# ai4ce/V2X-Sim

Measured on AMD Instinct MI355X. Metric: BEV frames/sec, V2VNet 5-agent detection (256x256 BEV), higher is better.
Workload: dtype bf16

## Files before the change

v2x-sim_amd/csrc/conv_stream.hip:

```cpp
#include "conv_stream.h"
#include <cstdlib>
#include <type_traits>



#ifndef V2X_STREAM_PSWZ_BUILD
#define V2X_STREAM_PSWZ_BUILD 1
#endif
constexpr int PSH = V2X_STREAM_PSWZ_BUILD;
#ifndef V2X_STREAM_LSS_BUILD
#define V2X_STREAM_LSS_BUILD 1
#endif

template <int BCO>
constexpr int chain_lds_bytes() { return BCO * BCO * 2 + 2 * BCO * 4; }

template <int BCO, int NT>
__device__ __forceinline__ void stage_chain(const StreamArgs &a, char *cl) {
    constexpr int NKS = BCO / 32;
    for (int p = threadIdx.x; p < BCO * BCO / 8; p += NT) {
        const int row = p / (BCO / 8), c8 = p - row * (BCO / 8);
        const int i2 = row >> 4, fj = row & 15, ks = c8 >> 2, fq = c8 & 3;
        *reinterpret_cast<uint4 *>(cl + (((i2 * NKS + ks) * 4 + fq) * 16 + fj) * 16) =
            *reinterpret_cast<const uint4 *>(a.w2 + (size_t)row * BCO + c8 * 8);
// ... 305 lines not shown
        const bool first = kc < nc0;
        const bool hf = first && a.up0;
        int d = hf ? pd_half[0] : pd_full[0];
#pragma unroll
        for (int u = 1; u < 6; ++u) d = (t == u) ? (hf ? pd_half[u] : pd_full[u]) : d;
        glds16s(patch_src(a.in0, a.C0, a.in1, a.C1, nc0, kc, zero_page, d), s_patch + buf * PATCH_BYTES + (wave + 4 * t) * 1024);
    };
    auto issue_dummy = [&]() { glds16s(zero_page, s_dummy); };

#pragma unroll
    for (int t = 0; t < 6; ++t) issue_patch_piece(kc_lo, t, 0);
    issue_weights(0);
    issue_weights(1);
    issue_weights(2);

    f32x4_t acc[TCO][4];
#pragma unroll
    for (int i = 0; i < TCO; ++i)
#pragma unroll
        for (int f = 0; f < 4; ++f) acc[i][f] = (f32x4_t){0.f, 0.f, 0.f, 0.f};

    int s = 0;
    for (int kc = kc_lo; kc < kc_hi; ++kc) {
        const char *pb = s_patch + ((kc - kc_lo) & 1) * PATCH_BYTES;
        const bool half = (kc < nc0) && a.up0;
        const int sh = half ? 1 : 0, row_bytes = (half ? PW0 : PW) * 64;
#pragma unroll 1
        for (int ky = 0; ky < 3; ++ky) {
            int rowoff[4];
#pragma unroll
            for (int f = 0; f < 4; ++f) rowoff[f] = (((frow[f] + ky - sh) >> sh) + sh) * row_bytes;
#pragma unroll
            for (int kx = 0; kx < 3; ++kx, ++s) {
                const int tap = ky * 3 + kx;
                if (s + 3 >= S) wait_vmcnt<0>();
                else if (s < 2) { if (NW == 2) wait_vmcnt<4>(); else wait_vmcnt<2>(); }
                else { if (NW == 2) wait_vmcnt<6>(); else wait_vmcnt<4>(); }
                __builtin_amdgcn_s_barrier();
                if (s + 3 < S) {
                    issue_weights(s + 3);
                    if (tap < 6 && kc + 1 < kc_hi) issue_patch_piece(kc + 1, tap, (kc + 1 - kc_lo) & 1);
                    else issue_dummy();
                }
                const char *ws = s_ring + (s & (RING - 1)) * SLICE_BYTES;
                bf16x8_t fa[TCO], fb[4];
#pragma unroll
                for (int f = 0; f < 4; ++f)
                    fb[f] = *reinterpret_cast<const bf16x8_t *>(pb + rowoff[f] + (half ? ct_half[f][kx] : ct_full[f][kx]));
#pragma unroll
                for (int i = 0; i < TCO; ++i)
                    fa[i] = *reinterpret_cast<const bf16x8_t *>(ws + (fq * BCO + i * 16 + fj) * 16);
#pragma unroll
                for (int i = 0; i < TCO; ++i)
#pragma unroll
                    for (int f = 0; f < 4; ++f)
                        acc[i][f] = __builtin_amdgcn_mfma_f32_16x16x32_bf16(fa[i], fb[f], acc[i][f], 0, 0, 0);

                __builtin_amdgcn_sched_group_barrier(0x100, TCO + 4, 0);
                __builtin_amdgcn_sched_group_barrier(0x008, TCO * 4, 0);
            }
        }
    }

    if constexpr (SPLITK) {
        const size_t npix = (size_t)a.N * a.H * a.W;
#pragma unroll
        for (int i = 0; i < TCO; ++i)
#pragma unroll
            for (int f = 0; f < 4; ++f) {
                const size_t pix = (size_t)(n * a.H + y0 + frow[f]) * a.W + x0 + ((TW == 32) ? (f & 1) * 16 + fj : fj);
                *reinterpret_cast<f32x4_t *>(a.ws + ((size_t)blockIdx.y * npix + pix) * a.w_rows + co_tile * BCO + i * 16 + fq * 4) = acc[i][f];
            }
    } else {
        stream_epilogue<BCO, TW, EPI, 4, false, true, true>(a, acc, co_tile, n, y0, x0, frow, fj, fq, nullptr, nullptr, 0, a.x4 != 0);
    }
}

template <bool GRU>
__global__ __launch_bounds__(256) void splitk_reduce_kernel(const float *__restrict__ ws, int ksplit, long long npix, int w_rows, int Cout,
                                                            const float *__restrict__ scale, const float *__restrict__ shift, int relu,
                                                            uint16_t *__restrict__ out, int out_cstride, int out_coff) {
    const int quads = Cout / 4;
    const long long total = npix * quads;
    for (long long t = (long long)blockIdx.x * 256 + threadIdx.x; t < total; t += (long long)gridDim.x * 256) {
        const long long pix = t / quads;
        const int c = (int)(t - pix * quads) * 4;
        if constexpr (GRU) {
            const int row = (c >> 5) * 96 + ((c >> 4) & 1) * 48 + (c & 15);
            f32x4_t g[3];
#pragma unroll
            for (int q = 0; q < 3; ++q) g[q] = (f32x4_t){0.f, 0.f, 0.f, 0.f};
            for (int sp = 0; sp < ksplit; ++sp)
#pragma unroll
                for (int q = 0; q < 3; ++q) g[q] += *reinterpret_cast<const f32x4_t *>(ws + ((size_t)sp * npix + pix) * w_rows + row + 16 * q);
            float h[4];
#pragma unroll
            for (int r = 0; r < 4; ++r) {
                const float4 b = reinterpret_cast<const float4 *>(scale)[c + r];
                h[r] = v2x_gru_h0(g[0][r], g[1][r], g[2][r], b);
            }
            uint2 o;
            o.x = pack_bf16x2(h[0], h[1]);
            o.y = pack_bf16x2(h[2], h[3]);
            *reinterpret_cast<uint2 *>(out + pix * out_cstride + out_coff + c) = o;
        } else {
            f32x4_t v = (f32x4_t){0.f, 0.f, 0.f, 0.f};
            for (int sp = 0; sp < ksplit; ++sp) v += *reinterpret_cast<const f32x4_t *>(ws + ((size_t)sp * npix + pix) * w_rows + c);
            const float4 sc = *reinterpret_cast<const float4 *>(scale + c), sf = *reinterpret_cast<const float4 *>(shift + c);
            uint2 o;
            o.x = pack_bf16x2(v[0] * sc.x + sf.x, v[1] * sc.y + sf.y);
            o.y = pack_bf16x2(v[2] * sc.z + sf.z, v[3] * sc.w + sf.w);
            if (relu) {
                o.x = v2x_relu_bf16x2(o.x);
                o.y = v2x_relu_bf16x2(o.y);
            }
            *reinterpret_cast<uint2 *>(out + pix * out_cstride + out_coff + c) = o;
        }
    }
}


template <int BCO, int EPI>
__global__ __launch_bounds__(512) __attribute__((amdgpu_waves_per_eu(2, 2))) void conv3x3_stream8_kernel(const StreamArgs a) {
    constexpr bool PERSIST = (EPI != SEPI_CHAIN);
    constexpr int TH = 16, TW = 32;
    constexpr int PW = TW + 2, PH = TH + 2, PW0 = TW / 2 + 2;
    constexpr int TCO = BCO / 16;
    constexpr int W_PIECES = BCO / 16;
    constexpr int SLICE_BYTES = BCO * 64;
    constexpr int N_ST = (EPI == SEPI_GRU) ? (TCO / 3) * 4 : TCO * 4;
    static_assert(PH * PW * 4 <= (PATCH8_PIECES - 1) * 64, "patch must leave the last piece as padding");
    static_assert(W_PIECES <= 8, "at most one weight DMA per wave per step");
    static_assert(4 + N_ST <= 63, "vmcnt is a 6-bit counter");

    extern __shared__ __attribute__((aligned(16))) char smem[];
    char *s_ring = smem;
    char *s_patch = smem + RING * SLICE_BYTES;
    char *s_dummy = s_patch + (PATCH8_PIECES - 1) * 1024;

    const int tid = threadIdx.x;
    const int lane = tid & 63;
    const int wave = __builtin_amdgcn_readfirstlane(tid >> 6);
    const int grp = wave >> 2, wv = wave & 3;
    const int fj = lane & 15, fq = lane >> 4;

    const int nwg = gridDim.x;
    const int bid = xcd_major_bid(blockIdx.x, nwg);
    const int n_tiles = a.n_px_tiles * a.n_co_tiles;
    const int co_tile = bid % a.n_co_tiles;
    const int txy = a.tiles_x * a.tiles_y;

    const int nc0 = a.C0 >> 5, nchunks = (a.C0 + a.C1) >> 5;
    const int S = nchunks * 9;
    const uint16_t *wbase = a.w + (size_t)co_tile * nchunks * 9 * (BCO * 32);
    const void *zero_page = a.w + (size_t)a.n_co_tiles * nchunks * 9 * (BCO * 32);
    char *s_chain = smem + RING * SLICE_BYTES + 2 * PATCH8_BYTES;
    if constexpr (EPI == SEPI_CHAIN) stage_chain<BCO, 512>(a, s_chain);

    auto tile_coords = [&](int t, int &n, int &y0, int &x0) { stream_tile_coords<TH, TW>(a.tiles_x, a.n_co_tiles, txy, t, n, y0, x0); };
    auto desc = [&](int n, int y0, int x0, int t, bool hf) -> int {
        return patch_desc<TH, TW, PSH>(a.H, a.W, n, y0, x0, (wave + 8 * t) * 64 + lane, hf);
    };

    int frow[4], ct[4][3];
#pragma unroll
    for (int f = 0; f < 4; ++f) frow[f] = 8 * grp + 2 * wv + (f >> 1);

    const bool has_w = wave < W_PIECES;
    const uint16_t *wsrc = wbase + lane * 8 + wave * 512;
    auto issue_dummy = [&]() { glds16s(zero_page, s_dummy); };
    auto issue_slice = [&](int slice, int slot, bool real) {
        if (has_w && real) glds16s(wsrc + (size_t)slice * (BCO * 32), s_ring + slot * SLICE_BYTES + wave * 1024);
        else issue_dummy();
    };
    auto issue_piece = [&](int d, int kc, int t, int buf) {
        glds16s(patch_src(a.in0, a.C0, a.in1, a.C1, nc0, kc, zero_page, d), s_patch + buf * PATCH8_BYTES + (wave + 8 * t) * 1024);
    };
    const bool chunk0_half = (nc0 > 0) && a.up0;

    int tile = bid;
    int n, y0, x0;
    tile_coords(tile, n, y0, x0);
    int pd[5];
    bool pd_half = chunk0_half;
#pragma unroll
    for (int t = 0; t < 5; ++t) pd[t] = desc(n, y0, x0, t, pd_half);

#pragma unroll
    for (int t = 0; t < 5; ++t) issue_piece(pd[t], 0, t, 0);
    issue_slice(0, 0, true); issue_dummy();
    issue_slice(1, 1, true); issue_dummy();
    issue_slice(2, 2, true); issue_dummy();
    wait_vmcnt<4>();
    __builtin_amdgcn_s_barrier();
    if (grp == 1) __builtin_amdgcn_s_barrier();

    int g = 0;
    int gc = 0;
    int relaxed = 0;
    for (;;) {
        const int next = tile + nwg;
        const bool has_next = PERSIST && next < n_tiles;
        int nn = 0, ny0 = 0, nx0 = 0;
        if (has_next) tile_coords(next, nn, ny0, nx0);

        f32x4_t acc[TCO][4];
#pragma unroll
        for (int i = 0; i < TCO; ++i)
#pragma unroll
            for (int f = 0; f < 4; ++f) acc[i][f] = (f32x4_t){0.f, 0.f, 0.f, 0.f};

        int s = 0;
        for (int kc = 0; kc < nchunks; ++kc, ++gc) {
            const char *pb = s_patch + (gc & 1) * PATCH8_BYTES;
            const bool half = (kc < nc0) && a.up0;
            const int sh = half ? 1 : 0, row_bytes = (half ? PW0 : PW) * 64;
            const bool last_chunk = kc + 1 == nchunks;
            const int kcn = last_chunk ? 0 : kc + 1;
            const bool fill = !last_chunk || has_next;
            const bool hfn = (kcn < nc0) && a.up0;
            if ((last_chunk && has_next) || (fill && hfn != pd_half)) {
                const int dn = last_chunk ? nn : n, dy = last_chunk ? ny0 : y0, dx = last_chunk ? nx0 : x0;
#pragma unroll
                for (int t = 0; t < 5; ++t) {
                    pd[t] = desc(dn, dy, dx, t, hfn);
                    __builtin_amdgcn_sched_barrier(0);
                }
                pd_half = hfn;
            }
            if (kc == 0 || kc == nc0) patch_col_table<4, TW, PSH>(ct, fj, fq, half);
#pragma unroll 1
            for (int ky = 0; ky < 3; ++ky) {
                int rowoff[4];
#pragma unroll
                for (int f = 0; f < 4; ++f) rowoff[f] = (((frow[f] + ky - sh) >> sh) + sh) * row_bytes;
#pragma unroll
                for (int kx = 0; kx < 3; ++kx, ++s, ++g) {
                    const int tap = ky * 3 + kx;
                    {
                        const int s3 = s + 3;
                        issue_slice(s3 < S ? s3 : s3 - S, (g + 3) & (RING - 1), s3 < S || has_next);
                    }
                    if (tap < 5 && fill) {
                        int d = pd[0];
#pragma unroll
                        for (int u = 1; u < 5; ++u) d = (tap == u) ? pd[u] : d;
                        issue_piece(d, kcn, tap, (gc + 1) & 1);
                    } else {
                        issue_dummy();
                    }
                    const char *ws = s_ring + (g & (RING - 1)) * SLICE_BYTES;
                    bf16x8_t fa[TCO], fb[4];
#pragma unroll
                    for (int f = 0; f < 4; ++f)
                        fb[f] = *reinterpret_cast<const bf16x8_t *>(pb + rowoff[f] + ct[f][kx]);
#pragma unroll
                    for (int i = 0; i < TCO; ++i)
                        fa[i] = *reinterpret_cast<const bf16x8_t *>(ws + (fq * BCO + i * 16 + fj) * 16);
                    if (relaxed > 0) {
                        wait_vmcnt<4 + N_ST>();
                        --relaxed;
                    } else {
                        wait_vmcnt<4>();
                    }
                    asm volatile("s_waitcnt lgkmcnt(0)" ::: "memory");
                    __builtin_amdgcn_sched_barrier(0);
                    __builtin_amdgcn_s_barrier();
                    __builtin_amdgcn_sched_barrier(0);
#pragma unroll
                    for (int i = 0; i < TCO; ++i)
#pragma unroll
                        for (int f = 0; f < 4; ++f)
                            acc[i][f] = __builtin_amdgcn_mfma_f32_16x16x32_bf16(fa[i], fb[f], acc[i][f], 0, 0, 0);
                    __builtin_amdgcn_sched_barrier(0);
                    __builtin_amdgcn_s_barrier();
                    __builtin_amdgcn_sched_barrier(0);
                }
            }
        }
        stream_epilogue<BCO, TW, EPI, 4, EPI == SEPI_CHAIN, true, EPI == SEPI_CHAIN>(a, acc, co_tile, n, y0, x0, frow, fj, fq, s_chain, nullptr, 0, a.x4 != 0);
        if (!has_next) break;
        tile = next;
        n = nn;
        y0 = ny0;
        x0 = nx0;
        relaxed = 2;
    }
    if (grp == 0) __builtin_amdgcn_s_barrier();
}

int v2x_conv_stream_pc_launch(const StreamArgs &a, hipStream_t s);

int v2x_num_cus() {
    static int n[V2X_MAX_DEVICES] = {0};
    int dev = 0, v = 0;
    if (hipGetDevice(&dev) != hipSuccess || dev < 0 || dev >= V2X_MAX_DEVICES) return 256;
    if (n[dev] == 0)
        n[dev] = (hipDeviceGetAttribute(&v, hipDeviceAttributeMultiprocessorCount, dev) == hipSuccess && v > 0) ? v : 256;
    return n[dev];
}

#define V2X_STREAM8G_ISSUE_DMAS \
                if (grp == 1) { \
                    const int ahead = st + 2; \
                    const int wslot = slot == 0 ? 2 : slot - 1; \
                    if (ahead < S3) nw = issue_weights(ahead, wslot, wv, 4); \
                    else if (has_next && ahead - S3 < S3) nw = issue_weights(ahead - S3, wslot, wv, 4); \
                } else if (fill && kx < 2) { \
                    const int npieces = hfn ? (PH0 * PW0 * 4 + 63) / 64 : PATCH8_PIECES; \
_Pragma("unroll") \
                    for (int t = 0; t < 5; ++t) { \
                        const int tt = kx * 5 + t; \
                        if (wv + 4 * tt >= npieces) break; \
                        int d = pd[0]; \
_Pragma("unroll") \
                        for (int u = 1; u < 10; ++u) d = (tt == u) ? pd[u] : d; \
                        issue_piece(d, kcn, tt, (gc + 1) & 1); \
                    } \
                }
template <int BCO, int EPI, bool WT = false>
__global__ __launch_bounds__(512) __attribute__((amdgpu_waves_per_eu(2, 2))) void conv3x3_stream8g_kernel(const StreamArgs a) {
    constexpr int TH = 16, TW = 32;
    constexpr int PW = TW + 2, PH = TH + 2, PW0 = TW / 2 + 2, PH0 = TH / 2 + 2;
    constexpr int TCO = BCO / 16, HCO = TCO / 2;
    constexpr int W_PIECES = BCO / 16;
    constexpr int SLICE_BYTES = BCO * 64;
    constexpr int STEP_BYTES = 3 * SLICE_BYTES;
    constexpr int NWD = (3 * W_PIECES + 3) / 4;
    static_assert(EPI != SEPI_CHAIN, "the chained epilogue stays on conv3x3_stream8_kernel (its operands need the LDS; from L2: +5.3 %)");
    static_assert(TCO % 2 == 0 && PH * PW * 4 <= (PATCH8_PIECES - 1) * 64, "half taps; patch fits its buffer");
    constexpr int AT = WT ? HCO : TCO;
    constexpr int NF = WT ? 8 : 4;
    constexpr int NB = WT ? 12 : 8;
    constexpr int BT = (HCO % 2 == 0) ? 2 : HCO;
    constexpr int N_ST = (EPI == SEPI_GRU) ? (TCO / 3) * 2 : TCO * 2;

    extern __shared__ __attribute__((aligned(16))) char smem[];
    char *s_ring = smem;
    char *s_patch = smem + 3 * STEP_BYTES;

    const int tid = threadIdx.x;
    const int lane = tid & 63;
    const int wave = __builtin_amdgcn_readfirstlane(tid >> 6);
    const int grp = wave >> 2, wv = wave & 3;
    const int fj = lane & 15, fq = lane >> 4;

    const int nwg = gridDim.x;
    int bid = xcd_major_bid(blockIdx.x, nwg);
    if (a.xcd_walk != 0 && a.n_co_tiles == 8 && (nwg & 7) == 0 && (nwg >> 3) == 32) {
        const int x = bid >> 5, i = bid & 31;
        bid = (((x >> 1) * 8 + (i >> 2)) << 3) + (x & 1) * 4 + (i & 3);
    }
    const int n_tiles = a.n_px_tiles * a.n_co_tiles;
    const int co_tile = bid % a.n_co_tiles;
    const int txy = a.tiles_x * a.tiles_y;
    const int nc0 = a.C0 >> 5, nchunks = (a.C0 + a.C1) >> 5;
    const int S3 = nchunks * 3;
    const uint16_t *wbase = a.w + (size_t)co_tile * nchunks * 9 * (BCO * 32);
    const void *zero_page = a.w + (size_t)a.n_co_tiles * nchunks * 9 * (BCO * 32);

    auto tile_coords = [&](int t, int &n, int &y0, int &x0) { stream_tile_coords<TH, TW>(a.tiles_x, a.n_co_tiles, txy, t, n, y0, x0); };
    auto desc = [&](int n, int y0, int x0, int t, bool hf) -> int {
        return patch_desc<TH, TW, PSH>(a.H, a.W, n, y0, x0, (wv + 4 * t) * 64 + fresh_lane(), hf);
    };
    auto issue_piece = [&](int d, int kc, int t, int buf) {
        glds16s_aux<V2X_STREAM8G_PATCH_AUX>(patch_src(a.in0, a.C0, a.in1, a.C1, nc0, kc, zero_page, d), s_patch + buf * PATCH8_BYTES + (wv + 4 * t) * 1024);
    };
    auto issue_weights = [&](int st, int slot, int wq, int NQ) -> int {
        const int kc = st / 3, kx = st - kc * 3;
        const int lane_w = fresh_lane();
        int cnt = 0;
#pragma unroll
        for (int u = 0; u < NWD; ++u) {
            const int p = wq + NQ * u;
            if (p >= 3 * W_PIECES) break;
            ++cnt;
            const int ky = p / W_PIECES, pis = p - ky * W_PIECES;
            glds16s_aux<V2X_STREAM8G_WEIGHT_AUX>(wbase + (size_t)(kc * 9 + ky * 3 + kx) * (BCO * 32) + pis * 512 + lane_w * 8,
                    s_ring + slot * STEP_BYTES + ky * SLICE_BYTES + pis * 1024);
        }
        return cnt;
    };
    auto wait_keep = [&](int keep, bool plus_stores) {
        if (plus_stores) {
            if (keep == NWD) asm volatile("s_waitcnt vmcnt(%0)" ::"n"(NWD + N_ST) : "memory");
            else if (keep == NWD - 1) asm volatile("s_waitcnt vmcnt(%0)" ::"n"(NWD - 1 + N_ST) : "memory");
            else asm volatile("s_waitcnt vmcnt(%0)" ::"n"(N_ST) : "memory");
        } else {
            if (keep == NWD) asm volatile("s_waitcnt vmcnt(%0)" ::"n"(NWD) : "memory");
            else if (keep == NWD - 1) asm volatile("s_waitcnt vmcnt(%0)" ::"n"(NWD - 1) : "memory");
            else asm volatile("s_waitcnt vmcnt(0)" ::: "memory");
        }
    };

    const int coh = WT ? (wv & 1) : 0;
    const int R0 = WT ? 8 * grp + 4 * (wv >> 1) : 8 * grp + 2 * wv;
    int frow[NF];
#pragma unroll
    for (int f = 0; f < NF; ++f) frow[f] = R0 + (f >> 1);
    const bool chunk0_half = (nc0 > 0) && a.up0;

    int tile = bid;
    int n, y0, x0;
    tile_coords(tile, n, y0, x0);
    int pd[10];
    bool pd_half = chunk0_half;
    if (grp == 0) {
#pragma unroll
        for (int t = 0; t < 10; ++t) pd[t] = desc(n, y0, x0, t, pd_half);
#pragma unroll
        for (int t = 0; t < 10; ++t) issue_piece(pd[t], 0, t, 0);
    }
    {
        constexpr int NP8 = (3 * W_PIECES + 7) / 8;
        for (int stp = 0; stp < (S3 > 1 ? 2 : 1); ++stp) {
            const int lane_w = fresh_lane();
#pragma unroll
            for (int u = 0; u < NP8; ++u) {
                const int p = wave + 8 * u;
                if (p >= 3 * W_PIECES) break;
                const int ky = p / W_PIECES, pis = p - ky * W_PIECES;
                glds16s_aux<V2X_STREAM8G_WEIGHT_AUX>(wbase + (size_t)((stp / 3) * 9 + ky * 3 + (stp % 3)) * (BCO * 32) + pis * 512 + lane_w * 8,
                        s_ring + stp * STEP_BYTES + ky * SLICE_BYTES + pis * 1024);
            }
        }
    }
    float *s_ss = reinterpret_cast<float *>(smem + 3 * STEP_BYTES + 2 * PATCH8_BYTES);
    if constexpr (V2X_STREAM_LSS_BUILD != 0 && EPI != SEPI_GRU) {
        if constexpr (EPI == SEPI_GRU) {
            constexpr int NH = BCO / 3;
            for (int i = tid; i < NH * 4; i += 512) {
                const int hc = co_tile * NH + (i >> 2);
                s_ss[i] = hc < a.Cout ? a.scale[(size_t)hc * 4 + (i & 3)] : 0.f;
            }
        } else {
            for (int i = tid; i < BCO; i += 512) {
                const int co = co_tile * BCO + i;
                s_ss[i] = co < a.Cout ? a.scale[co] : 0.f;
                s_ss[BCO + i] = co < a.Cout ? a.shift[co] : 0.f;
            }
        }
    }
    asm volatile("s_waitcnt vmcnt(0) lgkmcnt(0)" ::: "memory");
    __builtin_amdgcn_s_barrier();
    if (grp == 1) __builtin_amdgcn_s_barrier();

    int g = 0;
    bool relaxed = false;
    int slot = 0;
    int gc = 0;
    for (;;) {
        const int next = tile + nwg;
        const bool has_next = next < n_tiles;
        int nn = 0, ny0 = 0, nx0 = 0;
        if (has_next) tile_coords(next, nn, ny0, nx0);

        f32x4_t acc[AT][NF];
#pragma unroll
        for (int i = 0; i < AT; ++i)
#pragma unroll
            for (int f = 0; f < NF; ++f) acc[i][f] = (f32x4_t)(0.f);

        for (int kc = 0; kc < nchunks; ++kc, ++gc) {
            const char *pb = s_patch + (gc & 1) * PATCH8_BYTES;
            const bool half = (kc < nc0) && a.up0;
            const bool last_chunk = kc + 1 == nchunks;
            const int kcn = last_chunk ? 0 : kc + 1;
            const bool fill = !last_chunk || has_next;
            const bool hfn = (kcn < nc0) && a.up0;
            if (grp == 0 && ((last_chunk && has_next) || (fill && hfn != pd_half))) {
                const int dn = last_chunk ? nn : n, dy = last_chunk ? ny0 : y0, dx = last_chunk ? nx0 : x0;
#pragma unroll
                for (int t = 0; t < 10; ++t) {
                    pd[t] = desc(dn, dy, dx, t, hfn);
                    __builtin_amdgcn_sched_barrier(0);
                }
                pd_half = hfn;
            }
            const int sh = half ? 1 : 0;
            const int row_bytes = (half ? PW0 : PW) * 64;
            const int row0 = (R0 >> sh) * row_bytes;
#pragma unroll 1
            for (int kx = 0; kx < 3; ++kx, ++g, slot = (slot == 2 ? 0 : slot + 1)) {
                const int st = kc * 3 + kx;
                const int ln = fresh_lane();
                const int fjl = ln & 15, fql = ln >> 4;
                int nw = 0;
                V2X_STREAM8G_ISSUE_DMAS
                __builtin_amdgcn_sched_barrier(0);
                bf16x8_t B[NB];
#pragma unroll
                for (int ch = 0; ch < 2; ++ch) {
                    const int col = ch * 16 + fjl + kx;
                    const int pc = ((col - sh) >> sh) + sh;
                    const int coff = ((pc << 2) + (fql ^ ((pc >> PSH) & 3))) * 16;
#pragma unroll
                    for (int q = 0; q < NB / 2; ++q) {
                        B[q * 2 + ch] = *reinterpret_cast<const bf16x8_t *>(pb + row0 + (((q - sh) >> sh) + sh) * row_bytes + coff);
                    }
                }
                const char *ws = s_ring + slot * STEP_BYTES + (fql * BCO + fjl) * 16 + coh * (HCO * 256);
                bf16x8_t A[2][WT ? BT : HCO];
#pragma unroll
                for (int i = 0; i < (WT ? BT : HCO); ++i) A[0][i] = *reinterpret_cast<const bf16x8_t *>(ws + i * 256);
                __builtin_amdgcn_s_waitcnt(0xc07f);
                if (grp == 1) {
                    wait_keep(nw, relaxed);
                    relaxed = false;
                } else if (kx == 2) {
                    asm volatile("s_waitcnt vmcnt(0)" ::: "memory");
                }
                __builtin_amdgcn_sched_barrier(0);
                __builtin_amdgcn_s_barrier();
                __builtin_amdgcn_sched_barrier(0);
                if constexpr (WT) {
                    constexpr int NBLK = 3 * HCO / BT;
#pragma unroll
                    for (int b = 0; b < NBLK; ++b) {
                        const int ky = (b * BT) / HCO, i0 = (b * BT) % HCO;
                        auto mma_tiles = [&](int j0, int j1) __attribute__((always_inline)) {
#pragma unroll
                            for (int j = j0; j < j1; ++j)
#pragma unroll
                                for (int f = 0; f < 8; ++f)
                                    acc[i0 + j][f] = __builtin_amdgcn_mfma_f32_16x16x32_bf16(A[b & 1][j], B[((f >> 1) + ky) * 2 + (f & 1)], acc[i0 + j][f], 0, 0, 0);
                        };
                        __builtin_amdgcn_sched_barrier(0);
                        mma_tiles(0, 1);
                        __builtin_amdgcn_sched_barrier(0);
                        if (b + 1 < NBLK) {
                            const int ky1 = ((b + 1) * BT) / HCO, j1 = ((b + 1) * BT) % HCO;
#pragma unroll
                            for (int j = 0; j < BT; ++j) A[(b + 1) & 1][j] = *reinterpret_cast<const bf16x8_t *>(ws + ky1 * SLICE_BYTES + (j1 + j) * 256);
                        }
                        __builtin_amdgcn_sched_barrier(0);
                        mma_tiles(1, BT);
                        __builtin_amdgcn_sched_barrier(0);
                    }
                } else {
                constexpr int H1 = 1;
#pragma unroll
                for (int h = 0; h < 6; ++h) {
                    const int ky = h >> 1, hh = h & 1;
                    auto mma_part = [&](int i0, int i1) __attribute__((always_inline)) {
#pragma unroll
                        for (int i = i0; i < i1; ++i)
#pragma unroll
                            for (int f = 0; f < 4; ++f)
                                acc[hh * HCO + i][f] = __builtin_amdgcn_mfma_f32_16x16x32_bf16(A[h & 1][i], B[((f >> 1) + ky) * 2 + (f & 1)], acc[hh * HCO + i][f], 0, 0, 0);
                    };
                    __builtin_amdgcn_sched_barrier(0);
                    mma_part(0, H1);
                    __builtin_amdgcn_sched_barrier(0);
                    if (h + 1 < 6) {
                        const int ky1 = (h + 1) >> 1, hh1 = (h + 1) & 1;
#pragma unroll
                        for (int i = 0; i < HCO; ++i) A[(h + 1) & 1][i] = *reinterpret_cast<const bf16x8_t *>(ws + ky1 * SLICE_BYTES + (hh1 * HCO + i) * 256);
                    }
                    __builtin_amdgcn_sched_barrier(0);
                    mma_part(H1, HCO);
                    __builtin_amdgcn_sched_barrier(0);
                }
                }
                __builtin_amdgcn_sched_barrier(0);
                __builtin_amdgcn_s_barrier();
                __builtin_amdgcn_sched_barrier(0);
            }
        }
        constexpr bool LSS = V2X_STREAM_LSS_BUILD != 0 && EPI != SEPI_GRU;
        if constexpr (WT)
            stream_epilogue<BCO / 2, TW, EPI, 8, false, true, true>(a, acc, co_tile * 2 + coh, n, y0, x0, frow, fj, fq, nullptr,
                                                                    LSS ? (lds_cf_t *)s_ss + coh * (EPI == SEPI_GRU ? 4 * (BCO / 6) : BCO / 2) : (lds_cf_t *)nullptr, BCO, a.x4 != 0);
        else stream_epilogue<BCO, TW, EPI, 4, false, true, true>(a, acc, co_tile, n, y0, x0, frow, fj, fq, nullptr, LSS ? (lds_cf_t *)s_ss : (lds_cf_t *)nullptr, BCO, a.x4 != 0);
        if (!has_next) break;
        tile = next;
        n = nn;
        y0 = ny0;
        x0 = nx0;
        relaxed = true;
    }
    if (grp == 0) __builtin_amdgcn_s_barrier();
}

template <int BCO, int EPI, bool WT = false>
static int launch_stream8g(const StreamArgs &a, hipStream_t s) {
    constexpr int smem = 3 * 3 * BCO * 64 + 2 * PATCH8_BYTES + 1024;
    static_assert(smem <= 160 * 1024, "LDS budget");
    const int n_tiles = a.n_px_tiles * a.n_co_tiles;
    int grid = n_tiles;
    int g = v2x_num_cus() / a.n_co_tiles * a.n_co_tiles;
    if (g > 0 && g < n_tiles) grid = g;
    return v2x_launch<conv3x3_stream8g_kernel<BCO, EPI, WT>>("conv3x3_stream8g_kernel", dim3(grid), dim3(512), smem, s, a);
}

template <int BCO, int EPI>
static int launch_stream8(const StreamArgs &a, hipStream_t s) {
    constexpr int smem = RING * BCO * 64 + 2 * PATCH8_BYTES + (EPI == SEPI_CHAIN ? chain_lds_bytes<BCO>() : 0);
    const int n_tiles = a.n_px_tiles * a.n_co_tiles;
    int grid = n_tiles;
    if (v2x_tune(V2X_TUNE_STREAM_PERSIST) != 0) {
        int g = v2x_num_cus() / a.n_co_tiles * a.n_co_tiles;
        if (EPI != SEPI_CHAIN && g > 0 && g < n_tiles && ((a.C0 + a.C1) >> 5) >= 2) grid = g;
    }
    return v2x_launch<conv3x3_stream8_kernel<BCO, EPI>>("conv3x3_stream8_kernel", dim3(grid), dim3(512), smem, s, a);
}

constexpr int WPATCH_PIECES = 39;
constexpr int WPATCH_BYTES = WPATCH_PIECES * 1024;

template <int BCO, int EPI>
__global__ __launch_bounds__(256) __attribute__((amdgpu_waves_per_eu(2, 2))) void conv3x3_wide_kernel(const StreamArgs a) {
    constexpr int TH = 16, TW = 32, NF = 8;
    constexpr int PW = TW + 2, PH = TH + 2, PW0 = TW / 2 + 2, PH0 = TH / 2 + 2;
    constexpr int TCO = BCO / 16;
    constexpr int SLICE_BYTES = BCO * 64;
    constexpr int PPW = (WPATCH_PIECES + 3) / 4;
    static_assert(BCO == 64, "wide form: one 64-row channel tile (1 weight DMA per wave and step)");
    static_assert(PH * PW * 4 <= WPATCH_PIECES * 64, "patch must fit its buffer");

    extern __shared__ __attribute__((aligned(16))) char smem[];
    char *s_ring = smem;
    char *s_patch = smem + RING * SLICE_BYTES;

    const int tid = threadIdx.x;
    const int lane = tid & 63;
    const int wave = __builtin_amdgcn_readfirstlane(tid >> 6);
    const int fj = lane & 15, fq = lane >> 4;

    const int bid = xcd_major_bid(blockIdx.x, gridDim.x);
    int co_tile, n, y0, x0;
    stream_tile_coords<TH, TW>(a.tiles_x, a.tiles_y, a.n_co_tiles, bid, co_tile, n, y0, x0);

    const int nc0 = a.C0 >> 5, nchunks = (a.C0 + a.C1) >> 5;
    const int S = nchunks * 9;
    const uint16_t *wbase = a.w + (size_t)co_tile * nchunks * 9 * (BCO * 32);
    const void *zero_page = a.w + (size_t)a.n_co_tiles * nchunks * 9 * (BCO * 32);
    char *s_chain = smem + RING * SLICE_BYTES + WPATCH_BYTES;
    if constexpr (EPI == SEPI_CHAIN) stage_chain<BCO, 256>(a, s_chain);

    int pd[PPW];
    auto build_pd = [&](bool hf) {
        int lane_o = lane;
        asm volatile("" : "+v"(lane_o));
#pragma unroll
        for (int t = 0; t < PPW; ++t) {
            pd[t] = patch_desc<TH, TW, PSH>(a.H, a.W, n, y0, x0, (wave + 4 * t) * 64 + lane_o, hf);
            __builtin_amdgcn_sched_barrier(0);
        }
    };
    int frow[NF], ct[2][3];
#pragma unroll
    for (int f = 0; f < NF; ++f) frow[f] = 4 * wave + (f >> 1);

    const uint16_t *wsrc = wbase + lane * 8 + wave * 512;
    auto issue_weights = [&](int s) {
        glds16s(wsrc + (size_t)s * (BCO * 32), s_ring + (s & (RING - 1)) * SLICE_BYTES + wave * 1024);
    };
    auto issue_patch = [&](int kc, bool hf) {
        const bool first = kc < nc0;
        const uint16_t *src = first ? a.in0 : a.in1;
        const unsigned cs = first ? (unsigned)a.C0 : (unsigned)a.C1;
        const int npieces = hf ? (PH0 * PW0 * 4 + 63) / 64 : WPATCH_PIECES;
#pragma unroll
        for (int t = 0; t < PPW; ++t) {
            if (wave + 4 * t >= npieces) break;
            int d = pd[t];
            asm volatile("" : "+v"(d));
            glds16s(patch_src(src, cs, first ? kc : kc - nc0, zero_page, d), s_patch + (wave + 4 * t) * 1024);
        }
    };

    f32x4_t acc[TCO][NF];
#pragma unroll
    for (int i = 0; i < TCO; ++i)
#pragma unroll
        for (int f = 0; f < NF; ++f) acc[i][f] = (f32x4_t){0.f, 0.f, 0.f, 0.f};

    issue_weights(0);
    issue_weights(1);
    issue_weights(2);

    int s = 0;
    bool cur_half = false;
    for (int kc = 0; kc < nchunks; ++kc) {
        const bool half = (kc < nc0) && a.up0;
        const int sh = half ? 1 : 0, row_bytes = (half ? PW0 : PW) * 64;
        if (kc == 0 || half != cur_half) {
            build_pd(half);
            patch_col_table<2, TW, PSH>(ct, fj, fq, half);
            cur_half = half;
        }
        if (kc > 0) __builtin_amdgcn_s_barrier();
        issue_patch(kc, half);
        wait_vmcnt<0>();
        __builtin_amdgcn_s_barrier();
#pragma unroll 1
        for (int ky = 0; ky < 3; ++ky) {
            int rowoff[NF / 2];
#pragma unroll
            for (int r = 0; r < NF / 2; ++r) rowoff[r] = (((4 * wave + r + ky - sh) >> sh) + sh) * row_bytes;
#pragma unroll
            for (int kx = 0; kx < 3; ++kx, ++s) {
                const int tap = ky * 3 + kx;
                if (tap > 0) {
                    if (s + 2 >= S) wait_vmcnt<0>();
                    else wait_vmcnt<2>();
                    __builtin_amdgcn_s_barrier();
                }
                if (s + 3 < S) issue_weights(s + 3);
                const char *ws = s_ring + (s & (RING - 1)) * SLICE_BYTES;
                bf16x8_t fa[TCO], fb[NF];
#pragma unroll
                for (int f = 0; f < NF; ++f) fb[f] = *reinterpret_cast<const bf16x8_t *>(s_patch + rowoff[f >> 1] + ct[f & 1][kx]);
#pragma unroll
                for (int i = 0; i < TCO; ++i)
                    fa[i] = *reinterpret_cast<const bf16x8_t *>(ws + (fq * BCO + i * 16 + fj) * 16);
#pragma unroll
                for (int i = 0; i < TCO; ++i)
#pragma unroll
                    for (int f = 0; f < NF; ++f)
                        acc[i][f] = __builtin_amdgcn_mfma_f32_16x16x32_bf16(fa[i], fb[f], acc[i][f], 0, 0, 0);
                __builtin_amdgcn_sched_group_barrier(0x100, TCO + NF, 0);
                __builtin_amdgcn_sched_group_barrier(0x008, TCO * NF, 0);
            }
        }
    }
    stream_epilogue<BCO, TW, EPI, NF, EPI == SEPI_CHAIN, true, true>(a, acc, co_tile, n, y0, x0, frow, fj, fq, s_chain, nullptr, 0, a.x4 != 0);
}

template <int BCO>
__global__ __launch_bounds__(256) __attribute__((amdgpu_waves_per_eu(2, 2))) void conv3x3_wide3_kernel(const StreamArgs a) {
    constexpr int TH = 16, TW = 32, NF = 8, NB = 12;
    constexpr int PW = TW + 2, PW0 = TW / 2 + 2, PH0 = TH / 2 + 2;
    constexpr int TCO = BCO / 16;
    constexpr int SLICE_BYTES = BCO * 64, STEP_BYTES = 3 * SLICE_BYTES;
    constexpr int PPW = (WPATCH_PIECES + 3) / 4;
    static_assert(BCO == 64, "wide form: one 64-row channel tile (one weight piece per wave and tap)");

    extern __shared__ __attribute__((aligned(16))) char smem[];
    char *s_ring = smem;
    char *s_patch = smem + 3 * STEP_BYTES;

    const int tid = threadIdx.x;
    const int lane = tid & 63;
    const int wave = __builtin_amdgcn_readfirstlane(tid >> 6);
    const int fj = lane & 15, fq = lane >> 4;

    const int bid = xcd_major_bid(blockIdx.x, gridDim.x);
    int co_tile, n, y0, x0;
    stream_tile_coords<TH, TW>(a.tiles_x, a.tiles_y, a.n_co_tiles, bid, co_tile, n, y0, x0);

    const int nc0 = a.C0 >> 5, nchunks = (a.C0 + a.C1) >> 5;
    const int S3 = nchunks * 3;
    const uint16_t *wbase = a.w + (size_t)co_tile * nchunks * 9 * (BCO * 32);
    const void *zero_page = a.w + (size_t)a.n_co_tiles * nchunks * 9 * (BCO * 32);

    int pd[PPW];
    auto build_pd = [&](bool hf) {
        int lane_o = lane;
        asm volatile("" : "+v"(lane_o));
#pragma unroll
        for (int t = 0; t < PPW; ++t) {
            pd[t] = patch_desc<TH, TW, PSH>(a.H, a.W, n, y0, x0, (wave + 4 * t) * 64 + lane_o, hf);
            __builtin_amdgcn_sched_barrier(0);
        }
    };
    int frow[NF], ct[2][3];
#pragma unroll
    for (int f = 0; f < NF; ++f) frow[f] = 4 * wave + (f >> 1);

    const uint16_t *wsrc = wbase + lane * 8 + wave * 512;
    auto issue_weights = [&](int st) {
        const int kc = st / 3, kx = st - kc * 3;
        const int slot = st % 3;
#pragma unroll
        for (int ky = 0; ky < 3; ++ky)
            glds16s(wsrc + (size_t)(kc * 9 + ky * 3 + kx) * (BCO * 32), s_ring + slot * STEP_BYTES + ky * SLICE_BYTES + wave * 1024);
    };
    auto issue_patch = [&](int kc, bool hf) {
        const bool first = kc < nc0;
        const uint16_t *src = first ? a.in0 : a.in1;
        const unsigned cs = first ? (unsigned)a.C0 : (unsigned)a.C1;
        const int npieces = hf ? (PH0 * PW0 * 4 + 63) / 64 : WPATCH_PIECES;
#pragma unroll
        for (int t = 0; t < PPW; ++t) {
            if (wave + 4 * t >= npieces) break;
            int d = pd[t];
            asm volatile("" : "+v"(d));
            glds16s(patch_src(src, cs, first ? kc : kc - nc0, zero_page, d), s_patch + (wave + 4 * t) * 1024);
        }
    };

    f32x4_t acc[TCO][NF];
#pragma unroll
    for (int i = 0; i < TCO; ++i)
#pragma unroll
        for (int f = 0; f < NF; ++f) acc[i][f] = (f32x4_t){0.f, 0.f, 0.f, 0.f};

    issue_weights(0);
    issue_weights(1);

    int st = 0;
    bool cur_half = false;
    for (int kc = 0; kc < nchunks; ++kc) {
        const bool half = (kc < nc0) && a.up0;
        const int sh = half ? 1 : 0, row_bytes = (half ? PW0 : PW) * 64;
        if (kc == 0 || half != cur_half) {
            build_pd(half);
            patch_col_table<2, TW, PSH>(ct, fj, fq, half);
            cur_half = half;
// ... 195 lines not shown
```

Baseline: 6554.

## Specialise the BCO=96 stream8g kx loop with unrolled, precomputed LDS addressing

For the 96-channel tile the kx loop is fully unrolled and the weight ring slot is fixed to kx. Patch column offsets are precomputed into a per-lane table and row offsets are made wave-uniform with readfirstlane. Weight DMA addressing is simplified to contiguous per-chunk slices, and the vmcnt waits are specialised to match. The aim is to cut per-iteration address arithmetic and fresh_lane calls in the inner loop, at the cost of more registers and code size, with some risk to the prefetch/wait ordering.

Result: faster. 6628, median of 6 (+1.1%).

```diff
diff --git a/v2x-sim_amd/csrc/conv_stream.hip b/v2x-sim_amd/csrc/conv_stream.hip
--- a/v2x-sim_amd/csrc/conv_stream.hip
+++ b/v2x-sim_amd/csrc/conv_stream.hip
@@ -631,10 +631,14 @@
 
 #define V2X_STREAM8G_ISSUE_DMAS \
                 if (grp == 1) { \
-                    const int ahead = st + 2; \
-                    const int wslot = slot == 0 ? 2 : slot - 1; \
-                    if (ahead < S3) nw = issue_weights(ahead, wslot, wv, 4); \
-                    else if (has_next && ahead - S3 < S3) nw = issue_weights(ahead - S3, wslot, wv, 4); \
+                    if constexpr (LP96) { \
+                        if (kx == 0 || fill) nw = issue_weights96(kx == 0 ? wc0 : wc1, (kx + 2) % 3); \
+                    } else { \
+                        const int ahead = st + 2; \
+                        const int wslot = slot == 0 ? 2 : slot - 1; \
+                        if (ahead < S3) nw = issue_weights(ahead, wslot, wv, 4); \
+                        else if (has_next && ahead - S3 < S3) nw = issue_weights(ahead - S3, wslot, wv, 4); \
+                    } \
                 } else if (fill && kx < 2) { \
                     const int npieces = hfn ? (PH0 * PW0 * 4 + 63) / 64 : PATCH8_PIECES; \
 _Pragma("unroll") \
@@ -663,6 +667,8 @@
     constexpr int NB = WT ? 12 : 8;
     constexpr int BT = (HCO % 2 == 0) ? 2 : HCO;
     constexpr int N_ST = (EPI == SEPI_GRU) ? (TCO / 3) * 2 : TCO * 2;
+    constexpr bool LP96 = (BCO == 96);
+    constexpr int KXU = LP96 ? 3 : 1;
 
     extern __shared__ __attribute__((aligned(16))) char smem[];
     char *s_ring = smem;
@@ -709,6 +715,19 @@
                     s_ring + slot * STEP_BYTES + ky * SLICE_BYTES + pis * 1024);
         }
         return cnt;
+    };
+    const unsigned wl_off = LP96 ? (unsigned)((wv * 64 + lane) * 16) : 0u;
+    auto woff96 = [&](int u) -> int { return ((wv + 4 * u) / W_PIECES) * (2 * SLICE_BYTES) + u * 4096; };
+    const int nw96 = LP96 ? (3 * W_PIECES - wv + 3) / 4 : 0;
+    auto issue_weights96 = [&](const uint16_t *chunk_w, int kxa) -> int {
+        const char *src = reinterpret_cast<const char *>(chunk_w) + kxa * SLICE_BYTES;
+        char *dst = s_ring + kxa * STEP_BYTES + wv * 1024;
+#pragma unroll
+        for (int u = 0; u < NWD; ++u) {
+            if (u >= nw96) break;
+            glds16s_aux<V2X_STREAM8G_WEIGHT_AUX>(src + woff96(u) + wl_off, dst + u * 4096);
+        }
+        return nw96;
     };
     auto wait_keep = [&](int keep, bool plus_stores) {
         if (plus_stores) {
@@ -728,6 +747,10 @@
 #pragma unroll
     for (int f = 0; f < NF; ++f) frow[f] = R0 + (f >> 1);
     const bool chunk0_half = (nc0 > 0) && a.up0;
+    int ct[2][3];
+    bool ct_half = chunk0_half;
+    if constexpr (LP96) patch_col_table<2, TW, PSH>(ct, fj, fq, ct_half);
+    const int a_off96 = LP96 ? (fq * BCO + fj) * 16 + coh * (HCO * 256) : 0;
 
     int tile = bid;
     int n, y0, x0;
@@ -809,10 +832,22 @@
             const int sh = half ? 1 : 0;
             const int row_bytes = (half ? PW0 : PW) * 64;
             const int row0 = (R0 >> sh) * row_bytes;
-#pragma unroll 1
+            const uint16_t *wc0 = LP96 ? wbase + (size_t)kc * 9 * (BCO * 32) : wbase;
+            const uint16_t *wc1 = LP96 ? wbase + (size_t)kcn * 9 * (BCO * 32) : wbase;
+            int pbrow = 0, rq[NB / 2] = {};
+            if constexpr (LP96) {
+                if (half != ct_half) {
+                    patch_col_table<2, TW, PSH>(ct, fj, fq, half);
+                    ct_half = half;
+                }
+                pbrow = __builtin_amdgcn_readfirstlane(3 * STEP_BYTES + (gc & 1) * PATCH8_BYTES + row0);
+#pragma unroll
+                for (int q = 0; q < NB / 2; ++q) rq[q] = __builtin_amdgcn_readfirstlane((((q - sh) >> sh) + sh) * row_bytes);
+            }
+#pragma unroll KXU
             for (int kx = 0; kx < 3; ++kx, ++g, slot = (slot == 2 ? 0 : slot + 1)) {
                 const int st = kc * 3 + kx;
-                const int ln = fresh_lane();
+                const int ln = LP96 ? 0 : fresh_lane();
                 const int fjl = ln & 15, fql = ln >> 4;
                 int nw = 0;
                 V2X_STREAM8G_ISSUE_DMAS
@@ -820,21 +855,37 @@
                 bf16x8_t B[NB];
 #pragma unroll
                 for (int ch = 0; ch < 2; ++ch) {
-                    const int col = ch * 16 + fjl + kx;
-                    const int pc = ((col - sh) >> sh) + sh;
-                    const int coff = ((pc << 2) + (fql ^ ((pc >> PSH) & 3))) * 16;
-#pragma unroll
-                    for (int q = 0; q < NB / 2; ++q) {
-                        B[q * 2 + ch] = *reinterpret_cast<const bf16x8_t *>(pb + row0 + (((q - sh) >> sh) + sh) * row_bytes + coff);
+                    if constexpr (LP96) {
+                        const int c0 = ct[ch][kx] + pbrow;
+#pragma unroll
+                        for (int q = 0; q < NB / 2; ++q) B[q * 2 + ch] = *reinterpret_cast<const bf16x8_t *>(smem + (c0 + rq[q]));
+                    } else {
+                        const int col = ch * 16 + fjl + kx;
+                        const int pc = ((col - sh) >> sh) + sh;
+                        const int coff = ((pc << 2) + (fql ^ ((pc >> PSH) & 3))) * 16;
+#pragma unroll
+                        for (int q = 0; q < NB / 2; ++q) {
+                            B[q * 2 + ch] = *reinterpret_cast<const bf16x8_t *>(pb + row0 + (((q - sh) >> sh) + sh) * row_bytes + coff);
+                        }
                     }
                 }
-                const char *ws = s_ring + slot * STEP_BYTES + (fql * BCO + fjl) * 16 + coh * (HCO * 256);
+                const char *ws = LP96 ? s_ring + kx * STEP_BYTES + a_off96
+                                      : s_ring + slot * STEP_BYTES + (fql * BCO + fjl) * 16 + coh * (HCO * 256);
                 bf16x8_t A[2][WT ? BT : HCO];
 #pragma unroll
                 for (int i = 0; i < (WT ? BT : HCO); ++i) A[0][i] = *reinterpret_cast<const bf16x8_t *>(ws + i * 256);
                 __builtin_amdgcn_s_waitcnt(0xc07f);
                 if (grp == 1) {
-                    wait_keep(nw, relaxed);
+                    if constexpr (LP96) {
+                        if (nw != 0 && !relaxed) {
+                            if (nw96 == NWD) asm volatile("s_waitcnt vmcnt(%0)" ::"n"(NWD) : "memory");
+                            else asm volatile("s_waitcnt vmcnt(%0)" ::"n"(NWD - 1) : "memory");
+                        } else {
+                            wait_keep(nw, relaxed);
+                        }
+                    } else {
+                        wait_keep(nw, relaxed);
+                    }
                     relaxed = false;
                 } else if (kx == 2) {
                     asm volatile("s_waitcnt vmcnt(0)" ::: "memory");
```
